# maxim2266/csvplus

Hardware: AMD Instinct MI355X
Metric: joined rows/sec (IndexOn build + chained Join, 1e8-row 3-col orders) (higher is better)
Workload: dtype u32; 1 GPU; BASELINE configs[3]: orders(1e8 x {cust_id,prod_id,qty}).Join(UniqueIndexOn customers.id 1e7).Join(UniqueIndexOn products.prod_id 1e5); rows=100000000, customers=10000000, products=100000, rows_this_rank=100000000, exchange=none (1 GPU), output=sorted positions

## Files before the change

csvplus_amd/csrc/capi.hip:

```cpp
#include <algorithm>
#include <map>
#include <mutex>
#include <new>

#include "cph_internal.hpp"
#include "codec_device.hpp"

namespace cph {

constexpr size_t kGuardBytes = 256;
constexpr uint8_t kGuardByte = 0xA5;

Status DevicePool::alloc(size_t bytes, void** out) {
    std::lock_guard<std::recursive_mutex> lk(mu_);
    const size_t want = (bytes + (guard ? kGuardBytes : 0) + 255) & ~(size_t)255;
    int best = -1;
    for (int i = 0; i < (int)free_.size(); i++) {
        if (free_[i].cap >= want && free_[i].cap <= want * 2 + (1u << 20)) {
            if (best < 0 || free_[i].cap < free_[best].cap) best = i;
        }
    }
    Block b;
    bool from_slab = false;
    for (size_t i = 0; i < slab_free_.size(); i++)
// ... 468 lines not shown
}

static int32_t fail(cph_ctx* ctx, const Status& s) {
    if (ctx) ctx->err = s.msg;
    return s.code;
}

static Status enter(cph_ctx* ctx) {
    if (!ctx) return {CPH_ERR_INVALID, "ctx is NULL"};
    CPH_HIP_TRY(hipSetDevice(ctx->device));
    return {};
}

struct BuildJob {
    cph_index* ix = nullptr;
    int32_t nkeycols = 0;
    std::vector<DevBuf> staged;
    DevCol dcols[kMaxKeyCols];
    DevBuf stats_dev;
    const void* sample_host = nullptr;
    size_t scratch_off = 0;
    GroupSpec spec;
    bool small = false;
    SmallBufs sbufs;
    bool presplit = false;
    bool sampled = false;
    bool no_sample = false;
    bool unique = false;
    bool no_direct = false;
    bool side = false;
    bool spec_split = false;
    bool exact_split = false;
    bool no_split = false;
    uint32_t* miss = nullptr;
    uint32_t* cs_over = nullptr;
    DevBuf cs_codes;
};

static Status build_phase1(cph_ctx* ctx, const cph_strcol* keycols, int32_t nkeycols, BuildJob* job) {
    CPH_TRY(validate_cols(keycols, nkeycols));
    cph_index* ix = job->ix;
    ix->ctx = ctx;
    ix->nrows = keycols[0].nrows;
    ix->table_rows = ix->nrows;
    ix->nkeycols = nkeycols;
    job->nkeycols = nkeycols;
    CPH_TRY(stage_cols(ctx, keycols, nkeycols, &job->staged, job->dcols));
    job->small = small_build_applies(ctx, job->dcols, nkeycols, ix->nrows);
    if (!job->small && !job->no_split && nkeycols == 1 && !job->dcols[0].fixed_width && ix->nrows >= (1ull << 22)) {
        CPH_TRY(codec_try_split(ctx, job->dcols, 1, ix->nrows, nullptr, &ix->codec, !job->exact_split, &job->spec_split));
        job->presplit = ix->codec.has_split();
    }
    job->sampled = !job->small && !job->presplit && !job->no_sample && codec_sample_applies(ctx, job->dcols, nkeycols, ix->nrows);
    if (job->sampled) CPH_TRY(codec_sample_launch(ctx, job->dcols[0], ix->nrows, &job->sample_host));
    else if (!job->small && !job->presplit) CPH_TRY(codec_stats_launch(ctx, job->dcols, nkeycols, &job->stats_dev));
    return {};
}

static Status build_phase2(cph_ctx* ctx, BuildJob* job, const void* stats_host);
static Status job_arm_miss(cph_ctx* ctx, BuildJob* job) {
    job->miss = host_word(ctx);
    return job->miss ? Status{} : Status{CPH_ERR_HIP, "no pinned host memory for the report words of a build"};
}
static Status build_encode_sort(cph_ctx* ctx, BuildJob* job);

static size_t job_readback_bytes(const BuildJob& j) {
    return j.small ? sizeof(SmallResult) : (j.presplit || j.sampled) ? 0 : sizeof(ColStats) * (size_t)j.nkeycols;
}

static void build_run(cph_ctx* ctx, std::vector<BuildJob>& jobs, std::vector<Status>& status) {
    const size_t nj = jobs.size();
    auto fail_all = [&](const Status& s) {
        for (size_t i = 0; i < nj; i++)
            if (status[i].ok()) status[i] = s;
    };
    size_t total = 0;
    bool any_general = false;
    for (size_t i = 0; i < nj; i++) {
        jobs[i].scratch_off = total;
        total += job_readback_bytes(jobs[i]);
        total = (total + 63) & ~(size_t)63;
        if (status[i].ok() && !jobs[i].small) any_general = true;
    }
    Status s = ensure_pinned_scratch(ctx, total > 64 ? total : 64);
    if (!s.ok()) return fail_all(s);
    uint8_t* h = static_cast<uint8_t*>(ctx->pinned_scratch);
    for (size_t i = 0; i < nj; i++) {
        if (!status[i].ok()) continue;
        if (jobs[i].small) {
            SideStream on_side(ctx, jobs[i].side);
            status[i] = small_build_launch(ctx, jobs[i].dcols, jobs[i].nkeycols, jobs[i].ix->nrows, &jobs[i].sbufs,
                                           reinterpret_cast<SmallResult*>(h + jobs[i].scratch_off));
            continue;
        }
        if (jobs[i].presplit || jobs[i].sampled) continue;
        hipError_t e = hipMemcpyAsync(h + jobs[i].scratch_off, jobs[i].stats_dev.get(), job_readback_bytes(jobs[i]),
                                      hipMemcpyDeviceToHost, jobs[i].side ? ctx->side_stream : ctx->stream);
        if (e != hipSuccess) status[i] = {CPH_ERR_HIP, std::string("statistics read-back: ") + hipGetErrorString(e)};
    }
    bool any_side = false;
    for (size_t i = 0; i < nj; i++) any_side = any_side || jobs[i].side;
    auto sync_streams = [&]() {
        return hipStreamSynchronize(ctx->stream) == hipSuccess && (!any_side || hipStreamSynchronize(ctx->side_stream) == hipSuccess);
    };
    if (!sync_streams()) return fail_all({CPH_ERR_HIP, "hipStreamSynchronize failed"});
    ctx->pool.flush_deferred();
    std::vector<std::vector<uint8_t>> stats_host(nj);
    std::vector<size_t> retry;
    for (size_t i = 0; i < nj; i++) {
        if (!status[i].ok()) continue;
        if (jobs[i].small) {
            const SmallResult res = *reinterpret_cast<const SmallResult*>(h + jobs[i].scratch_off);
            bool not_small = false;
            status[i] = small_build_finish(ctx, jobs[i].ix, jobs[i].nkeycols, &jobs[i].sbufs, &res, &not_small);
            jobs[i].sbufs = SmallBufs{};
            if (status[i].ok() && not_small) retry.push_back(i);
            else if (status[i].ok()) index_plan_table(jobs[i].ix);
            continue;
        }
        if (jobs[i].sampled) {
            const uint8_t* sh = static_cast<const uint8_t*>(jobs[i].sample_host);
            stats_host[i].assign(sh, sh + codec_sample_bytes());
        } else if (!jobs[i].presplit) {
            stats_host[i].assign(h + jobs[i].scratch_off, h + jobs[i].scratch_off + job_readback_bytes(jobs[i]));
        }
    }
    for (size_t i = 0; i < nj; i++)
        if (status[i].ok() && !jobs[i].small) {
            SideStream on_side(ctx, jobs[i].side);
            status[i] = build_phase2(ctx, &jobs[i], stats_host[i].data());
        }
    std::vector<size_t> resplit;
    std::vector<size_t> resort;
    if (any_general) {
        s = ensure_pinned_scratch(ctx, 2 * sizeof(uint32_t) * nj + 64);
        if (!s.ok()) return fail_all(s);
        uint32_t* fd = static_cast<uint32_t*>(ctx->pinned_scratch);
        uint32_t* sm = fd + nj;
        for (size_t i = 0; i < nj; i++) {
            if (!status[i].ok() || jobs[i].small) continue;
            hipStream_t js = jobs[i].side ? ctx->side_stream : ctx->stream;
            fd[i] = 0xFFFFFFFFu;
            sm[i] = 0;
            if (!jobs[i].ix->first_dup_dev) continue;
            hipError_t e = hipMemcpyAsync(&fd[i], jobs[i].ix->first_dup_dev.get(), sizeof(uint32_t), hipMemcpyDeviceToHost, js);
            if (e != hipSuccess) status[i] = {CPH_ERR_HIP, std::string("first-duplicate read-back: ") + hipGetErrorString(e)};
        }
        if (!sync_streams()) return fail_all({CPH_ERR_HIP, "hipStreamSynchronize failed"});
        ctx->pool.flush_deferred();
        for (size_t i = 0; i < nj; i++) {
            if (!status[i].ok() || jobs[i].small) continue;
            cph_index* ix = jobs[i].ix;
            if (jobs[i].miss) sm[i] = *(volatile uint32_t*)jobs[i].miss;
            if (sm[i]) { jobs[i].cs_codes.reset(); jobs[i].cs_over = nullptr; resplit.push_back(i); continue; }
            if (jobs[i].cs_over && *(volatile uint32_t*)jobs[i].cs_over) { resort.push_back(i); continue; }
            jobs[i].cs_codes.reset();
            ix->first_dup = fd[i] != 0xFFFFFFFFu ? (uint64_t)fd[i] : UINT64_MAX;
            ix->first_dup_dev.reset();
            index_plan_table(ix);
        }
    }
    for (size_t i : resort) {
        BuildJob& j = jobs[i];
        cph_index* ix = j.ix;
        const uint64_t n = ix->nrows;
        uint32_t* over = j.cs_over;
        j.cs_over = nullptr;
        ix->sorted_codes.reset(); ix->perm.reset(); ix->first_dup_dev.reset();
        DevBuf kb, va, vb;
        Status r = kb.alloc(&ctx->pool, n * sizeof(uint32_t));
        if (r.ok()) r = va.alloc(&ctx->pool, n * sizeof(uint32_t));
        bool sorted_now = false;
        {
            CountedSortPlan first;
            int wb = counted_sort_plan(ctx, n, ix->codec.word_states[0], &first) ? (int)first.wbits : 0;
            for (int attempt = 0; attempt < 2 && r.ok() && !sorted_now && wb > 0; attempt++) {
                wb -= 2;
                CountedSortPlan csp;
                if (!counted_sort_plan(ctx, n, ix->codec.word_states[0], &csp, wb) || (int)csp.wbits != wb) break;
                r = ix->first_dup_dev.alloc(&ctx->pool, sizeof(uint32_t));
                if (r.ok()) r = counted_sort(ctx, csp, j.cs_codes.as<uint32_t>(), n, ix->codec.word_states[0], va.as<uint32_t>(), kb.as<uint32_t>(),
                                             ix->first_dup_dev.as<uint32_t>(), over);
                if (r.ok() && hipStreamSynchronize(ctx->stream) != hipSuccess) r = {CPH_ERR_HIP, "hipStreamSynchronize failed"};
                if (r.ok() && *(volatile uint32_t*)over == 0) {
                    ix->sorted_codes = std::move(kb);
                    ix->perm = std::move(va);
                    ix->sort_passes = 0;
                    r = index_first_dup_read(ctx, ix);
                    sorted_now = true;
                } else {
                    ix->first_dup_dev.reset();
                }
            }
        }
        if (sorted_now) {
            j.cs_codes.reset();
            if (r.ok()) index_plan_table(ix);
            status[i] = r;
            continue;
        }
        if (r.ok()) r = vb.alloc(&ctx->pool, n * sizeof(uint32_t));
        uint32_t *kout = nullptr, *vout = nullptr;
        int passes = 0;
        if (r.ok()) r = radix_sort_pairs<uint32_t>(ctx, j.cs_codes.as<uint32_t>(), kb.as<uint32_t>(), va.as<uint32_t>(), vb.as<uint32_t>(), true, n,
                                                   ix->codec.word_bits[0], &kout, &vout, &passes);
        if (r.ok()) {
            ix->sorted_codes = std::move(kout == j.cs_codes.as<uint32_t>() ? j.cs_codes : kb);
            ix->perm = std::move(vout == va.as<uint32_t>() ? va : vb);
            ix->sort_passes = passes;
            r = index_first_dup_launch(ctx, ix);
        }
        if (r.ok()) r = index_first_dup_read(ctx, ix);
        j.cs_codes.reset();
        if (r.ok()) index_plan_table(ix);
// ... 101 lines not shown
            w.seg_skip[w.nseg] = skip;
            w.seg_take[w.nseg] = t == left ? 0xFFFFFFFFu : t;
            w.nseg++;
            skip += t;
            left -= t;
            room -= t;
        } while (left > 0);
    }
    int total_words = 0;
    for (auto& w : W) {
        DevCol v[kMaxKeyCols];
        for (int s = 0; s < w.nseg; s++) v[s] = window_col(job->dcols, w, s);
        std::vector<ColStats> st;
        CPH_TRY(codec_collect_stats(ctx, v, w.nseg, &st));
        CPH_TRY(codec_build(st, &w.codec));
        w.codec.key32 = false;
        CPH_TRY(codec_upload(ctx, w.codec, &w.codec_dev));
        w.word_base = total_words;
        total_words += w.codec.nwords;
    }
    ix->codec = W[0].codec;
    DevBuf all, va, vb;
    CPH_TRY(all.alloc(&ctx->pool, (size_t)total_words * n * sizeof(uint64_t)));
    CPH_TRY(va.alloc(&ctx->pool, n * sizeof(uint32_t)));
    CPH_TRY(vb.alloc(&ctx->pool, n * sizeof(uint32_t)));
    std::vector<int> bits((size_t)total_words);
    for (auto& w : W) {
        DevCol v[kMaxKeyCols];
        for (int s = 0; s < w.nseg; s++) v[s] = window_col(job->dcols, w, s);
        CPH_TRY(codec_encode_build(ctx, w.codec, w.codec_dev, v, n, all.as<uint64_t>() + (uint64_t)w.word_base * n));
        for (int k = 0; k < w.codec.nwords; k++) bits[(size_t)(w.word_base + k)] = w.codec.word_bits[k];
    }
    CPH_TRY(sort_words_lsd(ctx, ix, all.as<uint64_t>(), total_words, bits.data(), n, va, vb));
    return index_first_dup_launch(ctx, ix);
}

static Status build_phase2(cph_ctx* ctx, BuildJob* job, const void* stats_host) {
    cph_index* ix = job->ix;
    const uint64_t n = ix->nrows;
    const int32_t nkeycols = job->nkeycols;
    const DevCol* dcols = job->dcols;
    if (job->presplit) {
        CPH_TRY(job_arm_miss(ctx, job));
        CPH_TRY(codec_upload(ctx, ix->codec, &ix->codec_dev));
        return build_encode_sort(ctx, job);
    }
    std::vector<ColStats> stats;
    if (job->sampled) {
        codec_sample_finish(dcols[0], stats_host, &stats);
        CPH_TRY(codec_build(stats, &ix->codec));
        if (codec_sample_checked(ix->codec, dcols)) {
            CPH_TRY(job_arm_miss(ctx, job));
            CPH_TRY(codec_upload(ctx, ix->codec, &ix->codec_dev));
            return build_encode_sort(ctx, job);
        }
        job->sampled = false;
        ix->codec = CodecHost{};
        CPH_TRY(codec_collect_stats(ctx, dcols, nkeycols, &stats));
    } else {
        codec_stats_finish(dcols, nkeycols, stats_host, &stats);
    }
    uint64_t positions = 0;
    for (const auto& s : stats) positions += s.maxlen;
    if (positions > (uint64_t)kMaxKeyBytes) return build_multi_window(ctx, job, stats);
    CPH_TRY(codec_build(stats, &ix->codec));
    if (!job->no_split) CPH_TRY(codec_try_split(ctx, dcols, nkeycols, n, &stats, &ix->codec));
    if (ix->codec.has_split()) {
        CPH_TRY(job_arm_miss(ctx, job));
    } else {
        CPH_TRY(codec_try_groups(ctx, dcols, nkeycols, n, &ix->codec, &job->spec));
    }
    CPH_TRY(codec_upload(ctx, ix->codec, &ix->codec_dev));
    return build_encode_sort(ctx, job);
}

static Status build_encode_sort(cph_ctx* ctx, BuildJob* job) {
    cph_index* ix = job->ix;
    const uint64_t n = ix->nrows;
    const DevCol* dcols = job->dcols;
    const CodecHost& cd = ix->codec;

    DevBuf va, vb;
    CPH_TRY(va.alloc(&ctx->pool, n * sizeof(uint32_t)));
    CPH_TRY(vb.alloc(&ctx->pool, n * sizeof(uint32_t)));
    int passes = 0;

    if (cd.nwords == 1) {
        const size_t kb_ = cd.key32 ? sizeof(uint32_t) : sizeof(uint64_t);
        DevBuf ka, kb, counts;
        CPH_TRY(ka.alloc(&ctx->pool, n * kb_));
        CPH_TRY(kb.alloc(&ctx->pool, n * kb_));
        const RadixPlan plan = radix_plan(ctx, n, cd.word_bits[0]);
        EncodeHist eh;
        const uint64_t states = cd.word_states[0];
        const bool direct = job->unique && !job->no_direct && ctx->direct_sort != 0 && cd.key32 && !job->spec.active && n >= (1ull << 16) &&
                            states >= n && states <= 2 * n && states < 0xFFFFFFFFull;
        if (direct) {
            if (!job->miss) {
                CPH_TRY(job_arm_miss(ctx, job));
            }
            DevBuf rt;
            uint64_t rt_blocks = 0;
            if (ctx->direct_ranktab && ctx->direct_sort == 1 && states != n && states <= (1ull << 30)) {
                rt_blocks = ranktab_blocks(states);
                if (!rt.alloc(&ctx->pool, rt_blocks * 8).ok()) rt_blocks = 0;
            }
            void* rtp = rt_blocks ? rt.get() : nullptr;
            ArithPlan ap;
            codec_arith_plan(cd, &ap);
            const DevCol& kc = dcols[0];
            if (ctx->direct_sort == 1 && ctx->direct_fused_encode && job->nkeycols == 1 && ap.enabled && ap.keylen == 8 && kc.fixed_width == 8 &&
                !kc.segmented() && ((uintptr_t)kc.data & 15) == 0) {
                CPH_TRY(direct_sort_windows_keys(ctx, reinterpret_cast<const uint64_t*>(kc.data), ap, n, states, va.as<uint32_t>(), ka.as<uint32_t>(),
                                                 job->miss, rtp, rt_blocks));
                ix->sorted_codes = std::move(ka);
                ix->perm = std::move(va);
                ix->sort_passes = 0;
                if (rtp) ix->ranktab = std::move(rt);
                return {};
            }
            CPH_TRY(codec_encode_build(ctx, cd, ix->codec_dev, dcols, n, ka.get(), &eh, nullptr, job->miss));
            CPH_TRY(direct_sort_windows(ctx, ka.as<uint32_t>(), n, states, va.as<uint32_t>(), ka.as<uint32_t>(), job->miss, rtp, rt_blocks));
            if (rtp) ix->ranktab = std::move(rt);
            ix->sorted_codes = std::move(ka);
            ix->perm = std::move(va);
            ix->sort_passes = 0;
            return {};
        }
        CountedSortPlan csp;
        if (cd.key32 && !job->spec.active && counted_sort_plan(ctx, n, states, &csp)) {
            uint32_t* over = host_word(ctx);
            if (!over) return {CPH_ERR_HIP, "no pinned host memory for the report words of a build"};
            vb.reset();
            CountedSort cs;
            CPH_TRY(cs.begin(ctx, csp, n));
            CPH_TRY(codec_encode_build(ctx, cd, ix->codec_dev, dcols, n, ka.get(), &eh, &job->spec, job->miss));
            CPH_TRY(ix->first_dup_dev.alloc(&ctx->pool, sizeof(uint32_t)));
            CPH_TRY(cs.run(ctx, ka.as<uint32_t>(), n, states, va.as<uint32_t>(), kb.as<uint32_t>(), ix->first_dup_dev.as<uint32_t>(), over, false));
            job->cs_over = over;
            job->cs_codes = std::move(ka);
            ix->sorted_codes = std::move(kb);
            ix->perm = std::move(va);
            ix->sort_passes = 0;
            return {};
        }
        if (plan.npass > 0) {
            CPH_TRY(counts.alloc(&ctx->pool, plan.count_words() * sizeof(uint32_t)));
            eh.tile_rows = plan.tile;
            eh.digit_mask = (1u << plan.nb0) - 1u;
            eh.bins = 1u << plan.rbits;
            eh.counts = counts.as<uint32_t>();
        }
        CPH_TRY(codec_encode_build(ctx, cd, ix->codec_dev, dcols, n, ka.get(), &eh, &job->spec, job->miss));
        if (job->spec.active) {
            uint32_t miss = 0;
            CPH_TRY(read_device_value(ctx, job->spec.miss.as<uint32_t>(), &miss));
            job->spec.active = false;
            if (miss) {
                const int bits_before = cd.word_bits[0];
                CPH_TRY(codec_groups_complete(ctx, dcols, job->nkeycols, n, miss, &job->spec, &ix->codec));
                CPH_TRY(codec_upload(ctx, ix->codec, &ix->codec_dev));
                if (cd.nwords != 1 || cd.word_bits[0] != bits_before || radix_plan(ctx, n, cd.word_bits[0]).npass != plan.npass) {
                    ka.reset(); kb.reset(); counts.reset(); va.reset(); vb.reset();
                    return build_encode_sort(ctx, job);
                }
                CPH_TRY(codec_encode_build(ctx, cd, ix->codec_dev, dcols, n, ka.get(), &eh, nullptr));
            }
        }
        uint32_t* vout;
        if (cd.key32) {
            uint32_t* kout;
            CPH_TRY(radix_sort_pairs<uint32_t>(ctx, ka.as<uint32_t>(), kb.as<uint32_t>(), va.as<uint32_t>(), vb.as<uint32_t>(),
                                               true, n, cd.word_bits[0], &kout, &vout, &passes, eh.counts, eh.done));
            ix->sorted_codes = std::move(kout == ka.as<uint32_t>() ? ka : kb);
        } else {
            uint64_t* kout;
            CPH_TRY(radix_sort_pairs<uint64_t>(ctx, ka.as<uint64_t>(), kb.as<uint64_t>(), va.as<uint32_t>(), vb.as<uint32_t>(),
                                               true, n, cd.word_bits[0], &kout, &vout, &passes, eh.counts, eh.done));
            ix->sorted_codes = std::move(kout == ka.as<uint64_t>() ? ka : kb);
        }
        ix->sort_passes = passes;
        ix->perm = std::move(vout == va.as<uint32_t>() ? va : vb);
    } else {
        DevBuf all;
        CPH_TRY(all.alloc(&ctx->pool, (size_t)cd.nwords * n * sizeof(uint64_t)));
        CPH_TRY(codec_encode_build(ctx, cd, ix->codec_dev, dcols, n, all.get(), nullptr, nullptr, job->miss));
        CPH_TRY(sort_words_lsd(ctx, ix, all.as<uint64_t>(), cd.nwords, cd.word_bits, n, va, vb));
    }

    CPH_TRY(index_first_dup_launch(ctx, ix));
    return {};
}

static Status index_build_impl(cph_ctx* ctx, const cph_strcol* keycols, int32_t nkeycols, cph_index* ix, bool unique) {
    if (nkeycols == 1 && keycols && keycols[0].mem == CPH_MEM_HOST && validate_cols(keycols, nkeycols).ok()) {
        bool taken = false;
        CPH_TRY(build_from_host_codes(ctx, keycols, nkeycols, ix, unique, &taken));
        if (taken) return {};
    }
    std::vector<BuildJob> jobs(1);
    std::vector<Status> st(1);
    jobs[0].ix = ix;
    jobs[0].unique = unique;
    st[0] = build_phase1(ctx, keycols, nkeycols, &jobs[0]);
    if (st[0].ok()) build_run(ctx, jobs, st);
    return st[0];
}

}

using namespace cph;

extern "C" {

CPH_API const char* cph_version(void) { return "csvplus_hip 0.1 (gfx950)"; }

CPH_API int32_t cph_ctx_create(int32_t device_id, cph_ctx** out) {
    if (!out) return CPH_ERR_INVALID;
    *out = nullptr;
    int count = 0;
    hipError_t e = hipGetDeviceCount(&count);
    if (e != hipSuccess || count <= 0) {
        (void)hipGetLastError();
        return CPH_ERR_NO_DEVICE;
    }
    if (device_id < 0 || device_id >= count) return CPH_ERR_NO_DEVICE;
    if (hipSetDevice(device_id) != hipSuccess) return CPH_ERR_NO_DEVICE;
    cph_ctx* ctx = new (std::nothrow) cph_ctx();
    if (!ctx) return CPH_ERR_NOMEM;
    ctx->device = device_id;
    if (hipStreamCreateWithFlags(&ctx->stream, hipStreamNonBlocking) != hipSuccess) {
        delete ctx;
        return CPH_ERR_HIP;
    }
    ctx->own_stream = true;
    warm_keycodec();
    warm_radix_sort();
    warm_probe();
    warm_chain();
    warm_materialize();
    warm_csv_ingest();
    warm_index_ops();
    warm_resolve();
    warm_small_build();
    warm_window_sort();
    warm_counted_sort();
    (void)ensure_pinned_scratch(ctx, 1 << 16);
    void* ring = nullptr;
    (void)pinned_upload(ctx, 64, &ring);
    (void)host_word(ctx);
    *out = ctx;
    return CPH_OK;
}

CPH_API void cph_ctx_destroy(cph_ctx* ctx) {
    if (!ctx) return;
    (void)hipSetDevice(ctx->device);
    (void)hipStreamSynchronize(ctx->stream);
    if (ctx->pinned_scratch) (void)hipHostFree(ctx->pinned_scratch);
    if (ctx->upload_ring) (void)hipHostFree(ctx->upload_ring);
    if (ctx->host_words) (void)hipHostFree(ctx->host_words);
    for (void* p : ctx->pinned_user) (void)hipHostFree(p);
    for (auto& b : ctx->pinned_user_free) (void)hipHostFree(b.first);
    for (auto& b : ctx->pinned_cache) (void)hipHostFree(b.first);
    for (auto& p : ctx->prof_pending) { (void)hipEventDestroy(p.start); (void)hipEventDestroy(p.stop); }
    for (hipEvent_t e : ctx->prof_free_events) (void)hipEventDestroy(e);
    hipStream_t own = ctx->own_stream ? ctx->stream : nullptr;
// ... 698 lines not shown
```

csvplus_amd/csrc/keycodec.hip:

```cpp
#include <algorithm>
#include <cmath>
#include <mutex>

#include "codec_device.hpp"
#include "host_encode_kernels.hpp"

namespace cph {

constexpr int kStatsThreads = 256;
constexpr int kStatsRows = 8;

template <class B, bool SEG>
__global__ __launch_bounds__(kStatsThreads) void k_col_stats(DevCol col, uint32_t* __restrict__ g_minmax,
                                                            uint32_t* __restrict__ g_mask) {
    __shared__ __attribute__((aligned(16))) uint8_t s_flag[kMaxKeyBytes * 256];
    __shared__ uint32_t s_min, s_max;
    {
        uint4* z = reinterpret_cast<uint4*>(s_flag);
        for (int i = threadIdx.x; i < kMaxKeyBytes * 256 / 16; i += kStatsThreads) z[i] = make_uint4(0, 0, 0, 0);
    }
    if (threadIdx.x == 0) { s_min = 0xFFFFFFFFu; s_max = 0; }
    __syncthreads();

    uint32_t mn = 0xFFFFFFFFu, mx = 0;
// ... 1219 lines not shown
        if (bits < best_bits) { best_bits = bits; best = (int)k; }
    }
    if (best < 0 || bits_sort_cost(plain_bits - most + best_bits) >= bits_sort_cost(plain_bits)) return -1;
    return best;
}

static std::vector<int> split_candidates(const SplitSample& hsm, uint64_t nsel) {
    std::vector<int> cand;
    for (int b = 0; b < 256; b++)
        if ((double)hsm.cnt[b] >= 0.99 * (double)nsel) cand.push_back(b);
    auto alnum = [](int b) { return (b >= '0' && b <= '9') || (b >= 'a' && b <= 'z') || (b >= 'A' && b <= 'Z'); };
    std::sort(cand.begin(), cand.end(), [&](int a, int b) { return alnum(a) != alnum(b) ? !alnum(a) : hsm.cnt[a] > hsm.cnt[b]; });
    if (cand.size() > 8) cand.resize(8);
    return cand;
}

static Status split_assemble(const cph_ctx* ctx, int c, int ncols, const std::vector<ColStats>* stats, uint32_t d, const SplitStats& st,
                             std::vector<WideKey>* dict_io, double plain_bits, CodecHost* out, bool* usable) {
    *usable = false;
    std::vector<WideKey>& dict = *dict_io;
    const uint32_t pmin = ~st.pmin_inv, smin = ~st.smin_inv;
    std::sort(dict.begin(), dict.end(), wide_less);

    std::vector<ColStats> vstats;
    for (int k = 0; k < ncols; k++) {
        if (k != c) { vstats.push_back((*stats)[(size_t)k]); continue; }
        ColStats pre{}, suf{};
        pre.minlen = pmin;
        pre.maxlen = st.pmax;
        for (uint32_t q = 0; q < st.pmax; q++) pre.mask[q][0] = 1u;
        suf.minlen = smin;
        suf.maxlen = st.smax;
        memcpy(suf.mask, st.mask, sizeof st.mask);
        vstats.push_back(pre);
        vstats.push_back(suf);
    }
    uint64_t positions = 0;
    for (const auto& v : vstats) positions += v.maxlen;
    if (positions > (uint64_t)kMaxKeyBytes || st.pmax == 0) return {};
    CodecHost trial;
    CPH_TRY(codec_build(vstats, &trial));
    const int p0 = trial.col_start[c];
    trial.unit.assign((size_t)trial.npos, kUnitPos);
    trial.dict_off.assign((size_t)trial.npos, 0);
    trial.dict_len.assign((size_t)trial.npos, 0);
    trial.unit[(size_t)p0] = kUnitWide;
    trial.radix[(size_t)p0] = (uint16_t)dict.size();
    for (int sym = 0; sym < kLutStride; sym++) trial.lut[(size_t)p0 * kLutStride + (size_t)sym] = kLutInvalid;
    for (uint32_t i = 1; i < st.pmax; i++) {
        trial.unit[(size_t)p0 + i] = kUnitAbsorbed;
        trial.radix[(size_t)p0 + i] = 1;
        for (int sym = 0; sym < kLutStride; sym++) trial.lut[((size_t)p0 + i) * kLutStride + (size_t)sym] = 0;
    }
    trial.split_col = c;
    trial.split_byte = (uint8_t)d;
    trial.split_maxlen = (int32_t)st.vmax;
    trial.wdict = std::move(dict);
    if (!codec_wide_perfect_hash(&trial)) return {};
    CPH_TRY(codec_split_words(&trial));
    if (ctx->codec_debug)
        fprintf(stderr, "codec_try_split: column %d cut at 0x%02x: %zu prefixes (<= %u bytes), suffix %u..%u bytes: %d word(s), %d bits, sort cost %.0f (plain: %.1f bits%s)\n",
                c, d, trial.wdict.size(), st.pmax, smin, st.smax, trial.nwords, trial.word_bits[0], codec_sort_cost(trial), plain_bits,
                stats ? "" : " by the sample");
    *out = std::move(trial);
    *usable = true;
    return {};
}

bool codec_sample_applies(const cph_ctx* ctx, const DevCol* cols, int32_t ncols, uint64_t n) {
    return ctx->stats_sample != 0 && ncols == 1 && cols[0].fixed_width >= 1 && cols[0].fixed_width <= (uint32_t)kSplitMaxValue &&
           !cols[0].segmented() && n >= (1ull << 20);
}
size_t codec_sample_bytes() { return sizeof(SplitSample); }
Status codec_sample_launch(cph_ctx* ctx, const DevCol& col, uint64_t n, const void** host_copy) {
    const uint64_t step = n >> 16;
    const uint64_t nsel = (n + step - 1) / step;
    DevBuf& acc = ctx->self_clean[ctx->stream_slot].sample;
    CPH_TRY(self_clean_block(ctx, &acc, sizeof(SplitSample) + 16));
    uint32_t* hw = host_word(ctx, (uint32_t)(sizeof(SplitSample) / 4));
    if (!hw) return {CPH_ERR_HIP, "no pinned host memory for the sample's statistics"};
    ProfScope ps(ctx, "k_split_count", 0);
    uint64_t nblk = (nsel + kSplitThreads - 1) / kSplitThreads;
    if (nblk > 1024) nblk = 1024;
    if (col.fixed_width <= 8)
        hipLaunchKernelGGL(k_sample_fixed8, dim3((unsigned)std::min<uint64_t>(nblk, (uint64_t)kFixed8Blocks)), dim3(kSplitThreads), 0, ctx->stream, col, step, nsel, acc.as<SplitSample>(),
                           reinterpret_cast<SplitSample*>(hw));
    else
        hipLaunchKernelGGL(k_split_count, dim3((unsigned)nblk), dim3(kSplitThreads), 0, ctx->stream, col, step, nsel, acc.as<SplitSample>(),
                           reinterpret_cast<SplitSample*>(hw));
    if (hipGetLastError() != hipSuccess) {
        acc.reset();
        return {CPH_ERR_HIP, "k_split_count launch failed"};
    }
    *host_copy = hw;
    return {};
}
void codec_sample_finish(const DevCol& col, const void* host_copy, std::vector<ColStats>* out) {
    const SplitSample* sm = static_cast<const SplitSample*>(host_copy);
    out->assign(1, ColStats{});
    ColStats& st = (*out)[0];
    st.minlen = st.maxlen = col.fixed_width;
    static_assert(sizeof(sm->mask) <= sizeof(st.mask), "the sample's positions must fit ColStats");
    memcpy(st.mask, sm->mask, sizeof sm->mask);
}
bool codec_sample_checked(const CodecHost& cd, const DevCol* cols) {
    return !cd.has_split() && !cd.has_groups() && cd.ncols == 1 && cd.nwords == 1 && codec_premultiplied_bits(cd) != 0 && !cols[0].segmented();
}

Status codec_try_split(cph_ctx* ctx, const DevCol* cols, int32_t ncols, uint64_t n, const std::vector<ColStats>* stats, CodecHost* codec,
                       bool speculate, bool* speculated) {
    if (speculated) *speculated = false;
    if (!ctx->codec_split || n < (1ull << 16) || ncols >= kMaxKeyCols) return {};
    if (stats && (codec->key32 || codec->has_groups())) return {};
    if (!stats && ncols != 1) return {};
    int c = -1;
    double most = 0, plain_bits = 0;
    if (stats) {
        for (int k = 0; k < ncols; k++) {
            double bits = 0;
            for (uint32_t q = 0; q < (*stats)[(size_t)k].maxlen; q++) bits += radix_bits((*stats)[(size_t)k], q);
            plain_bits += bits;
            if (cols[k].fixed_width || cols[k].segmented() || (*stats)[(size_t)k].maxlen > (uint32_t)kSplitMaxValue || (*stats)[(size_t)k].maxlen < 4) continue;
            if (bits > most) { most = bits; c = k; }
        }
        if (c < 0 || most < 24.0) return {};
    } else {
        if (cols[0].fixed_width || cols[0].segmented()) return {};
        c = 0;
    }
    const DevCol& col = cols[c];
    const uint64_t step = n > (1ull << 19) ? n >> 18 : 1;
    const uint64_t nsel = (n + step - 1) / step;

    DevBuf sample;
    CPH_TRY(sample.alloc(&ctx->pool, sizeof(SplitSample)));
    CPH_HIP_TRY(hipMemsetAsync(sample.get(), 0, sizeof(SplitSample), ctx->stream));
    {
        ProfScope ps(ctx, "k_split_count", 0);
        uint64_t nblk = (nsel + kSplitThreads - 1) / kSplitThreads;
        if (nblk > 1024) nblk = 1024;
        hipLaunchKernelGGL(k_split_count, dim3((unsigned)nblk), dim3(kSplitThreads), 0, ctx->stream, col, step, nsel, sample.as<SplitSample>(), (SplitSample*)nullptr);
        CPH_HIP_TRY(hipGetLastError());
    }
    CPH_TRY(ensure_pinned_scratch(ctx, sizeof(SplitSample)));
    CPH_HIP_TRY(hipMemcpyAsync(ctx->pinned_scratch, sample.get(), sizeof(SplitSample), hipMemcpyDeviceToHost, ctx->stream));
    CPH_HIP_TRY(hipStreamSynchronize(ctx->stream));
    std::vector<SplitSample> hsv(1);
    SplitSample& hsm = hsv[0];
    memcpy(&hsm, ctx->pinned_scratch, sizeof hsm);
    if (hsm.maxlen > (uint32_t)kSplitMaxValue || hsm.maxlen < 4) return {};
    if (!stats) {
        ColStats tmp{};
        tmp.minlen = ~hsm.minlen_inv;
        memcpy(tmp.mask, hsm.mask, sizeof hsm.mask);
        for (uint32_t q = 0; q < hsm.maxlen; q++) most += radix_bits(tmp, q);
        plain_bits = most;
        if (most <= 32.0) return {};
    }
    const bool small_values = (stats ? (*stats)[(size_t)c].maxlen : hsm.maxlen) <= 24;
    const std::vector<int> cand = split_candidates(hsm, nsel);
    if (cand.empty()) return {};

    const size_t set_bytes = (size_t)kSplitSetSlots * sizeof(SplitSlot);
    DevBuf sets, sstats;
    CPH_TRY(sets.alloc(&ctx->pool, cand.size() * set_bytes));
    CPH_TRY(sstats.alloc(&ctx->pool, cand.size() * sizeof(SplitStats)));
    CPH_HIP_TRY(hipMemsetAsync(sets.get(), 0, cand.size() * set_bytes, ctx->stream));
// ... 894 lines not shown
```

csvplus_amd/csrc/window_sort.hip:

```cpp
#include "cph_internal.hpp"
#include "codec_device.hpp"
#include "device_utils.hpp"

namespace cph {

constexpr int kWpThreads = 512;
constexpr int kWpItems = 16;
constexpr int kWpThreadsOneLevel = 1024;
constexpr int kWpItemsOneLevel = 8;
constexpr int kWpTile = kWpThreads * kWpItems;
static_assert(kWpThreadsOneLevel * kWpItemsOneLevel == kWpTile, "one tile size");
constexpr int kWpMaxBuckets = 2048;
constexpr int kWinBits = 14;
constexpr uint32_t kWinSlots = 1u << kWinBits;
constexpr uint32_t kWinEmpty = 0xFFFFFFFFu;
constexpr int kPlaceThreads = 512;

struct WpArgs {
    const uint64_t* keys;
    ArithPlan ap;
    const uint32_t* codes;
    const uint64_t* entries;
    const uint32_t* src_count;
    uint64_t n;
// ... 114 lines not shown
        uint32_t h[kWpMaxBuckets / THREADS], sum = 0;
#pragma unroll
        for (int k = 0; k < kWpMaxBuckets / THREADS; k++) {
            h[k] = (uint32_t)k < per ? s_hist[t * per + k] : 0u;
            sum += h[k];
        }
        uint32_t run = block_exclusive_sum<uint32_t, THREADS>(sum, s_tmp, &tot);
#pragma unroll
        for (int k = 0; k < kWpMaxBuckets / THREADS; k++) {
            if ((uint32_t)k < per) {
                const uint32_t b = t * per + k;
                s_start[b] = run;
                if (h[k]) s_delta[b] = atomicAdd(&a.dst_count[(uint64_t)sb * a.nb + b], h[k]) - run;
                run += h[k];
            }
        }
    }
    __syncthreads();
#pragma unroll
    for (int k = 0; k < ITEMS; k++)
        if (code[k] != kWinEmpty) s_ent[s_start[code[k] >> a.shift] + rank[k]] = ((uint64_t)code[k] << 32) | row[k];
    __syncthreads();
    const uint32_t cap = 1u << a.shift, mask = cap - 1u;
    bool over = false;
    uint64_t e[ITEMS];
    uint32_t pos[ITEMS];
#pragma unroll
    for (int k = 0; k < ITEMS; k++) {
        const uint32_t i = (uint32_t)k * THREADS + t;
        e[k] = s_ent[i < tot ? i : 0u];
    }
#pragma unroll
    for (int k = 0; k < ITEMS; k++) {
        const uint32_t i = (uint32_t)k * THREADS + t;
        pos[k] = s_delta[i < tot ? (uint32_t)(e[k] >> 32) >> a.shift : 0u] + i;
    }
#pragma unroll
    for (int k = 0; k < ITEMS; k++) {
        const uint32_t i = (uint32_t)k * THREADS + t;
        if (i < tot) {
            const uint32_t w = (uint32_t)(e[k] >> 32), b = w >> a.shift;
            if (pos[k] < cap) a.dst[(((uint64_t)sb * a.nb + b) << a.shift) + pos[k]] = ((uint64_t)(w & mask) << 32) | (uint32_t)e[k];
            else over = true;
        }
    }
    if (__ballot(over) && lane_id() == 0) *a.flag = 1u;
}

__global__ __launch_bounds__(1024) void k_win_offsets(const uint32_t* __restrict__ counts, uint32_t nwin, uint32_t* __restrict__ off) {
    __shared__ uint32_t s_tmp[1024 / kWave + 1];
    uint32_t carry = 0;
    for (uint32_t base = 0; base < nwin; base += 1024) {
        const uint32_t i = base + threadIdx.x;
        uint32_t v = i < nwin ? counts[i] : 0u;
        v = v < kWinSlots ? v : kWinSlots;
        uint32_t total;
        const uint32_t ex = block_exclusive_sum<uint32_t, 1024>(v, s_tmp, &total);
        if (i < nwin) off[i] = carry + ex;
        carry += total;
    }
}

__global__ __launch_bounds__(kPlaceThreads) void k_win_place(const uint64_t* __restrict__ entries, uint32_t* __restrict__ counts,
                                                            const uint32_t* __restrict__ off, uint64_t n, uint32_t* __restrict__ perm,
                                                            uint32_t* __restrict__ sorted, uint32_t* __restrict__ flag,
                                                            uint32_t* __restrict__ clear_also, uint32_t nclear, uint2* __restrict__ ranktab,
                                                            uint32_t rank_blocks) {
    extern __shared__ __attribute__((aligned(16))) uint8_t smem[];
    __shared__ uint32_t s_wcount[kPlaceThreads / kWave];
    typedef unsigned int u32x4 __attribute__((ext_vector_type(4)));
    uint32_t* win = reinterpret_cast<uint32_t*>(smem);
    const uint32_t g = blockIdx.x, t = threadIdx.x;
    const uint32_t craw = counts[g], cnt = craw < kWinSlots ? craw : kWinSlots;
    {
        u32x4 e;
        e.x = e.y = e.z = e.w = kWinEmpty;
        for (uint32_t i = t; i < kWinSlots / 4; i += kPlaceThreads) reinterpret_cast<u32x4*>(win)[i] = e;
    }
    __syncthreads();
    if (t == 0) {
        counts[g] = 0u;
        if (g < nclear) clear_also[g] = 0u;
    }
    const uint64_t* src = entries + ((uint64_t)g << kWinBits);
    for (uint32_t i = t; i < cnt; i += kPlaceThreads) {
        const uint64_t e = src[i];
        win[(uint32_t)(e >> 32) & (kWinSlots - 1u)] = (uint32_t)e;
    }
    __syncthreads();
    constexpr uint32_t kWaves = kPlaceThreads / kWave, kPerWave = kWinSlots / kWaves, kIters = kPerWave / kWave;
    const uint32_t wave = (uint32_t)wave_id(), lane = (uint32_t)lane_id();
    const uint32_t s0 = wave * kPerWave;
    uint32_t c = 0;
#pragma unroll 4
    for (uint32_t it = 0; it < kIters; it++) c += (uint32_t)__popcll(__ballot(win[s0 + it * kWave + lane] != kWinEmpty));
    if (lane == 0) s_wcount[wave] = c;
    __syncthreads();
    uint32_t before = 0, filled = 0;
#pragma unroll
    for (uint32_t w = 0; w < kWaves; w++) {
        const uint32_t x = s_wcount[w];
        before += w < wave ? x : 0u;
        filled += x;
    }
    if (t == 0 && (filled != craw)) *flag = 1u;
    uint64_t pos = (off ? (uint64_t)off[g] : ((uint64_t)g << kWinBits)) + before;
    const uint64_t lt = lanemask_lt();
    const uint32_t code0 = (g << kWinBits) + s0;
    for (uint32_t it = 0; it < kIters; it++) {
        const uint32_t v = win[s0 + it * kWave + lane];
        const uint64_t bal = __ballot(v != kWinEmpty);
        if (ranktab && lane < 2) {
            const uint32_t blk = ((code0 + it * kWave) >> 5) + lane;
            if (blk < rank_blocks)
                ranktab[blk] = make_uint2(lane ? (uint32_t)(bal >> 32) : (uint32_t)bal, (uint32_t)pos + (lane ? (uint32_t)__popc((uint32_t)bal) : 0u));
        }
        if (v != kWinEmpty) {
            const uint64_t p = pos + (uint64_t)__popcll(bal & lt);
            if (p < n) {
                perm[p] = v;
                sorted[p] = code0 + it * kWave + lane;
            }
        }
        pos += (uint64_t)__popcll(bal);
    }
}

Status WindowSort::begin(cph_ctx* ctx, uint64_t n_, uint64_t states_) {
    n = n_;
    states = states_;
    const uint64_t nwin = (states + kWinSlots - 1) >> kWinBits;
    two = nwin > (uint64_t)kWpMaxBuckets;
    int k2 = 0;
    if (two) {
        int wb = 0;
        while ((1ull << wb) < nwin) wb++;
        k2 = (wb + 1) / 2;
    }
    nb2 = 1u << k2;
    shift1 = (uint32_t)kWinBits + (uint32_t)k2;
    nb1 = two ? (states + (1ull << shift1) - 1) >> shift1 : nwin;
    if (nb1 > (uint64_t)kWpMaxBuckets) return {CPH_ERR_INVALID, "direct_sort_windows: code space too large"};
    nwin_total = two ? nb1 * nb2 : nwin;
    CPH_TRY(ent1.alloc(&ctx->pool, (nb1 << shift1) * sizeof(uint64_t)));
    if (two) CPH_TRY(ent2.alloc(&ctx->pool, (nwin_total << kWinBits) * sizeof(uint64_t)));
    const uint64_t nwords = nb1 + (two ? nwin_total : 0);
    words = &ctx->self_clean[ctx->stream_slot].win;
    CPH_TRY(self_clean_block(ctx, words, nwords * sizeof(uint32_t)));
    cur1 = words->as<uint32_t>();
    cur2 = two ? cur1 + nb1 : cur1;
    started = true;
    return {};
}
WindowSort::~WindowSort() {
    if (started && !finished && words) words->reset();
}

template <int SRC, int THREADS, int ITEMS>
static Status win_partition_launch(cph_ctx* ctx, const WpArgs& a, unsigned grid, double bytes) {
    const uint32_t nbp = (a.nb + (uint32_t)THREADS - 1u) & ~((uint32_t)THREADS - 1u);
    const size_t lds = (size_t)THREADS * ITEMS * 8 + (size_t)nbp * 12;
    CPH_TRY(kernel_setup(ctx, reinterpret_cast<const void*>(&k_win_partition<SRC, THREADS, ITEMS>), THREADS, lds, nullptr));
    ProfScope ps(ctx, "k_win_partition", bytes);
    hipLaunchKernelGGL((k_win_partition<SRC, THREADS, ITEMS>), dim3(grid), dim3(THREADS), lds, ctx->stream, a);
    return {};
}

Status WindowSort::add(cph_ctx* ctx, const uint32_t* codes, uint64_t row0, uint64_t m, uint32_t* flag, const uint64_t* keys, const ArithPlan* ap) {
    if (m == 0) return {};
    WpArgs a{};
// ... 87 lines not shown
```

Before: 142.6 billion rows/s.

## Split build sync per stream, defer sort buffer allocs, vectorize window place loads

Build completion now synchronizes the main and side streams separately and starts phase-2 for main-stream jobs before waiting on the side stream. It uses a cached pinned readback block when side streams are active. Allocation of the second value and key buffers and the radix plan is deferred until the path actually needs them, which avoids pool allocations on the direct and counted sort paths. The window place kernel now loads two 64-bit entries per 128-bit vector load with several loads in flight per thread. This adds some complexity and a clamped tail read.

```diff
diff --git a/csvplus_amd/csrc/capi.hip b/csvplus_amd/csrc/capi.hip
--- a/csvplus_amd/csrc/capi.hip
+++ b/csvplus_amd/csrc/capi.hip
@@ -574,9 +574,19 @@
         total = (total + 63) & ~(size_t)63;
         if (status[i].ok() && !jobs[i].small) any_general = true;
     }
-    Status s = ensure_pinned_scratch(ctx, total > 64 ? total : 64);
+    bool any_side = false;
+    for (size_t i = 0; i < nj; i++) any_side = any_side || jobs[i].side;
+    struct ReadbackBlock {
+        cph_ctx* c;
+        void* p = nullptr;
+        size_t cap = 0;
+        bool settled = false;
+        ~ReadbackBlock() { if (settled) pinned_cache_put(c, p, cap); }
+    } rb{ctx};
+    Status s = any_side ? pinned_cache_get(ctx, result_block_bytes(total > 64 ? total : 64), &rb.p, &rb.cap)
+                        : ensure_pinned_scratch(ctx, total > 64 ? total : 64);
     if (!s.ok()) return fail_all(s);
-    uint8_t* h = static_cast<uint8_t*>(ctx->pinned_scratch);
+    uint8_t* h = static_cast<uint8_t*>(any_side ? rb.p : ctx->pinned_scratch);
     for (size_t i = 0; i < nj; i++) {
         if (!status[i].ok()) continue;
         if (jobs[i].small) {
@@ -590,38 +600,40 @@
                                       hipMemcpyDeviceToHost, jobs[i].side ? ctx->side_stream : ctx->stream);
         if (e != hipSuccess) status[i] = {CPH_ERR_HIP, std::string("statistics read-back: ") + hipGetErrorString(e)};
     }
-    bool any_side = false;
-    for (size_t i = 0; i < nj; i++) any_side = any_side || jobs[i].side;
     auto sync_streams = [&]() {
         return hipStreamSynchronize(ctx->stream) == hipSuccess && (!any_side || hipStreamSynchronize(ctx->side_stream) == hipSuccess);
     };
-    if (!sync_streams()) return fail_all({CPH_ERR_HIP, "hipStreamSynchronize failed"});
-    ctx->pool.flush_deferred();
     std::vector<std::vector<uint8_t>> stats_host(nj);
     std::vector<size_t> retry;
-    for (size_t i = 0; i < nj; i++) {
-        if (!status[i].ok()) continue;
-        if (jobs[i].small) {
-            const SmallResult res = *reinterpret_cast<const SmallResult*>(h + jobs[i].scratch_off);
-            bool not_small = false;
-            status[i] = small_build_finish(ctx, jobs[i].ix, jobs[i].nkeycols, &jobs[i].sbufs, &res, &not_small);
-            jobs[i].sbufs = SmallBufs{};
-            if (status[i].ok() && not_small) retry.push_back(i);
-            else if (status[i].ok()) index_plan_table(jobs[i].ix);
-            continue;
-        }
-        if (jobs[i].sampled) {
-            const uint8_t* sh = static_cast<const uint8_t*>(jobs[i].sample_host);
-            stats_host[i].assign(sh, sh + codec_sample_bytes());
-        } else if (!jobs[i].presplit) {
-            stats_host[i].assign(h + jobs[i].scratch_off, h + jobs[i].scratch_off + job_readback_bytes(jobs[i]));
-        }
-    }
-    for (size_t i = 0; i < nj; i++)
-        if (status[i].ok() && !jobs[i].small) {
-            SideStream on_side(ctx, jobs[i].side);
-            status[i] = build_phase2(ctx, &jobs[i], stats_host[i].data());
-        }
+    for (int on = 0; on < (any_side ? 2 : 1); on++) {
+        if (hipStreamSynchronize(on ? ctx->side_stream : ctx->stream) != hipSuccess) return fail_all({CPH_ERR_HIP, "hipStreamSynchronize failed"});
+        if (!any_side) ctx->pool.flush_deferred();
+        for (size_t i = 0; i < nj; i++) {
+            if (!status[i].ok() || jobs[i].side != (on != 0)) continue;
+            if (jobs[i].small) {
+                const SmallResult res = *reinterpret_cast<const SmallResult*>(h + jobs[i].scratch_off);
+                bool not_small = false;
+                status[i] = small_build_finish(ctx, jobs[i].ix, jobs[i].nkeycols, &jobs[i].sbufs, &res, &not_small);
+                jobs[i].sbufs = SmallBufs{};
+                if (status[i].ok() && not_small) retry.push_back(i);
+                else if (status[i].ok()) index_plan_table(jobs[i].ix);
+                continue;
+            }
+            if (jobs[i].sampled) {
+                const uint8_t* sh = static_cast<const uint8_t*>(jobs[i].sample_host);
+                stats_host[i].assign(sh, sh + codec_sample_bytes());
+            } else if (!jobs[i].presplit) {
+                stats_host[i].assign(h + jobs[i].scratch_off, h + jobs[i].scratch_off + job_readback_bytes(jobs[i]));
+            }
+        }
+        for (size_t i = 0; i < nj; i++)
+            if (status[i].ok() && !jobs[i].small && jobs[i].side == (on != 0)) {
+                SideStream on_side(ctx, jobs[i].side);
+                status[i] = build_phase2(ctx, &jobs[i], stats_host[i].data());
+            }
+    }
+    rb.settled = true;
+    std::sort(retry.begin(), retry.end());
     std::vector<size_t> resplit;
     std::vector<size_t> resort;
     if (any_general) {
@@ -889,15 +901,12 @@
 
     DevBuf va, vb;
     CPH_TRY(va.alloc(&ctx->pool, n * sizeof(uint32_t)));
-    CPH_TRY(vb.alloc(&ctx->pool, n * sizeof(uint32_t)));
     int passes = 0;
 
     if (cd.nwords == 1) {
         const size_t kb_ = cd.key32 ? sizeof(uint32_t) : sizeof(uint64_t);
         DevBuf ka, kb, counts;
         CPH_TRY(ka.alloc(&ctx->pool, n * kb_));
-        CPH_TRY(kb.alloc(&ctx->pool, n * kb_));
-        const RadixPlan plan = radix_plan(ctx, n, cd.word_bits[0]);
         EncodeHist eh;
         const uint64_t states = cd.word_states[0];
         const bool direct = job->unique && !job->no_direct && ctx->direct_sort != 0 && cd.key32 && !job->spec.active && n >= (1ull << 16) &&
@@ -934,11 +943,11 @@
             ix->sort_passes = 0;
             return {};
         }
+        CPH_TRY(kb.alloc(&ctx->pool, n * kb_));
         CountedSortPlan csp;
         if (cd.key32 && !job->spec.active && counted_sort_plan(ctx, n, states, &csp)) {
             uint32_t* over = host_word(ctx);
             if (!over) return {CPH_ERR_HIP, "no pinned host memory for the report words of a build"};
-            vb.reset();
             CountedSort cs;
             CPH_TRY(cs.begin(ctx, csp, n));
             CPH_TRY(codec_encode_build(ctx, cd, ix->codec_dev, dcols, n, ka.get(), &eh, &job->spec, job->miss));
@@ -951,6 +960,8 @@
             ix->sort_passes = 0;
             return {};
         }
+        CPH_TRY(vb.alloc(&ctx->pool, n * sizeof(uint32_t)));
+        const RadixPlan plan = radix_plan(ctx, n, cd.word_bits[0]);
         if (plan.npass > 0) {
             CPH_TRY(counts.alloc(&ctx->pool, plan.count_words() * sizeof(uint32_t)));
             eh.tile_rows = plan.tile;
@@ -990,6 +1001,7 @@
         ix->perm = std::move(vout == va.as<uint32_t>() ? va : vb);
     } else {
         DevBuf all;
+        CPH_TRY(vb.alloc(&ctx->pool, n * sizeof(uint32_t)));
         CPH_TRY(all.alloc(&ctx->pool, (size_t)cd.nwords * n * sizeof(uint64_t)));
         CPH_TRY(codec_encode_build(ctx, cd, ix->codec_dev, dcols, n, all.get(), nullptr, nullptr, job->miss));
         CPH_TRY(sort_words_lsd(ctx, ix, all.as<uint64_t>(), cd.nwords, cd.word_bits, n, va, vb));
diff --git a/csvplus_amd/csrc/keycodec.hip b/csvplus_amd/csrc/keycodec.hip
--- a/csvplus_amd/csrc/keycodec.hip
+++ b/csvplus_amd/csrc/keycodec.hip
@@ -1325,7 +1325,7 @@
     ProfScope ps(ctx, "k_split_count", 0);
     uint64_t nblk = (nsel + kSplitThreads - 1) / kSplitThreads;
     if (nblk > 1024) nblk = 1024;
-    if (col.fixed_width <= 8)
+    if (col.fixed_width >= 1 && col.fixed_width <= 8)
         hipLaunchKernelGGL(k_sample_fixed8, dim3((unsigned)std::min<uint64_t>(nblk, (uint64_t)kFixed8Blocks)), dim3(kSplitThreads), 0, ctx->stream, col, step, nsel, acc.as<SplitSample>(),
                            reinterpret_cast<SplitSample*>(hw));
     else
diff --git a/csvplus_amd/csrc/window_sort.hip b/csvplus_amd/csrc/window_sort.hip
--- a/csvplus_amd/csrc/window_sort.hip
+++ b/csvplus_amd/csrc/window_sort.hip
@@ -220,10 +220,22 @@
         counts[g] = 0u;
         if (g < nclear) clear_also[g] = 0u;
     }
-    const uint64_t* src = entries + ((uint64_t)g << kWinBits);
-    for (uint32_t i = t; i < cnt; i += kPlaceThreads) {
-        const uint64_t e = src[i];
-        win[(uint32_t)(e >> 32) & (kWinSlots - 1u)] = (uint32_t)e;
+    constexpr uint32_t kPlaceLoads = 4, kRound = 2u * kPlaceLoads * kPlaceThreads;
+    const u32x4* src = reinterpret_cast<const u32x4*>(entries + ((uint64_t)g << kWinBits));
+    const uint32_t lastp = cnt ? (cnt - 1u) >> 1 : 0u;
+    for (uint32_t base = 0; base < cnt; base += kRound) {
+        u32x4 v[kPlaceLoads];
+#pragma unroll
+        for (uint32_t k = 0; k < kPlaceLoads; k++) {
+            const uint32_t p = (base >> 1) + k * kPlaceThreads + t;
+            v[k] = src[p < lastp ? p : lastp];
+        }
+#pragma unroll
+        for (uint32_t k = 0; k < kPlaceLoads; k++) {
+            const uint32_t i = base + 2u * (k * kPlaceThreads + t);
+            if (i < cnt) win[v[k].y & (kWinSlots - 1u)] = v[k].x;
+            if (i + 1u < cnt) win[v[k].w & (kWinSlots - 1u)] = v[k].z;
+        }
     }
     __syncthreads();
     constexpr uint32_t kWaves = kPlaceThreads / kWave, kPerWave = kWinSlots / kWaves, kIters = kPerWave / kWave;
```

Result: faster. 146.7 billion rows/s (median of 6 runs) (+2.9%).
